# ChrisTho23/DrakeGPT

Measured on NVIDIA B200. Metric: train_tokens_per_sec_TransformerLM_scaled, higher is better.
Workload: dtype bf16

## Files before the change

drakegpt_b200/csrc/attn_tc.cu:

```cuda
#include <cuda.h>

#include "common.cuh"
#include "ptx.cuh"

namespace dgpt {

using namespace ptx;

int make_tmap_bf16_2d(CUtensorMap* map, const void* base, int64_t inner, int64_t outer, int64_t ld, int box_outer);

static constexpr int HD = 64;
static constexpr int QT = 128;
static constexpr float kLog2e = 1.4426950408889634f;

struct AttnTcP {
  void *o, *dq, *dk, *dv;
  const void *o_in, *d_o;
  float* lse;
  int64_t o_rs, dq_rs, dk_rs, dv_rs, do_rs;
  int B, NH, T;
  float scale, inv_keep;
  uint32_t thr, site;
  uint64_t seed;
  const uint64_t* seed_dev;
};

__device__ __forceinline__ uint32_t pack_bf16(float a, float b) {
  __nv_bfloat162 v = __floats2bfloat162_rn(a, b);
  return *reinterpret_cast<uint32_t*>(&v);
}

__device__ __forceinline__ void store_row32_sw128(uint8_t* tile_base, int row, int c0, const float (&v)[32]) {
  uint8_t* blk = tile_base + (c0 >> 6) * 16384 + row * 128;
  const int chunk0 = (c0 & 63) >> 3;
#pragma unroll
  for (int j = 0; j < 4; ++j) {
    uint4 w;
    w.x = pack_bf16(v[8 * j], v[8 * j + 1]);
    w.y = pack_bf16(v[8 * j + 2], v[8 * j + 3]);
    w.z = pack_bf16(v[8 * j + 4], v[8 * j + 5]);
    w.w = pack_bf16(v[8 * j + 6], v[8 * j + 7]);
    *reinterpret_cast<uint4*>(blk + (((chunk0 + j) ^ (row & 7)) << 4)) = w;
  }
}

static constexpr int kFwd2Threads = 320;
static constexpr int kFwd2QK = 49152;
static constexpr int kFwd2Smem = 2 * kFwd2QK + 2 * 32768 + 256 + 1024;
static constexpr int kWHeavy = 5, kWLight = 2;

struct FwdSched {
  int nheavy, nlight;
  unsigned long long* probe;
};

__global__ void __launch_bounds__(kFwd2Threads, 1)
attn_fwd_tc2_kernel(const __grid_constant__ CUtensorMap map_q32, const __grid_constant__ CUtensorMap map_k,
                    const __grid_constant__ CUtensorMap map_v, AttnTcP p, FwdSched sc) {
  extern __shared__ uint8_t smem_raw[];
  uint8_t* smem = reinterpret_cast<uint8_t*>((reinterpret_cast<uintptr_t>(smem_raw) + 1023) & ~(uintptr_t)1023);
  uint8_t* sQK = smem;
  uint8_t* sV = smem + 2 * kFwd2QK;
  uint64_t* bars = reinterpret_cast<uint64_t*>(sV + 2 * 32768);
  uint64_t *qk_full = bars, *qk_empty = bars + 2, *v_full = bars + 4, *v_empty = bars + 6, *s_full = bars + 8,
           *p_full = bars + 10, *o_full = bars + 12, *slot_free = bars + 14;
  uint32_t* tmem_slot = reinterpret_cast<uint32_t*>(bars + 16);

  clock_probe_begin(sc.probe);
  const int warp = threadIdx.x >> 5, lane = threadIdx.x & 31;
  const int ntile = p.T / QT;

  const int G = gridDim.x, c = blockIdx.x;
  const int hq = sc.nheavy / G, hr = sc.nheavy % G;
  const int nh_c = hq + (c < hr ? 1 : 0);
  const int U = (kWHeavy * sc.nheavy + kWLight * sc.nlight + G - 1) / G;
  const int cap_hi = max(0, (U - kWHeavy * (hq + 1)) / kWLight), cap_lo = max(0, (U - kWHeavy * hq) / kWLight);
  const int cap_total = hr * cap_hi + (G - hr) * cap_lo;
  const int l_start = c < hr ? c * cap_hi : hr * cap_hi + (c - hr) * cap_lo;
  const int l0 = min(sc.nlight, l_start), l1 = min(sc.nlight, l_start + (c < hr ? cap_hi : cap_lo));
  const int n_extra = cap_total < sc.nlight ? (sc.nlight - cap_total - c + G - 1) / G : 0;
  const int n_items = nh_c + (l1 - l0) + max(0, n_extra);
  auto item = [&](int n, int& bh, int& qt) {
    if (n < nh_c) {
      const int hi = c + n * G;
      bh = hi; qt = ntile - 1;
    } else {
      const int m = n - nh_c;
      const int li = m < l1 - l0 ? l0 + m : cap_total + c + (m - (l1 - l0)) * G;
      bh = li; qt = 0;
    }
  };

  if (threadIdx.x == 0) {
    prefetch_tensormap(&map_q32);
    prefetch_tensormap(&map_k);
    prefetch_tensormap(&map_v);
    for (int g = 0; g < 2; ++g) {
      mbar_init(&qk_full[g], 1);
      mbar_init(&qk_empty[g], 1);
      mbar_init(&v_full[g], 1);
      mbar_init(&v_empty[g], 1);
      mbar_init(&s_full[g], 1);
      mbar_init(&p_full[g], 4);
      mbar_init(&o_full[g], 1);
      mbar_init(&slot_free[g], 4);
    }
    fence_barrier_init();
  }
  if (warp == 9) tmem_alloc<512>(tmem_slot);
  tc_fence_before();
  __syncthreads();
  tc_fence_after();
  const uint32_t tmem = *tmem_slot;
  pdl_grid_sync();

  if (warp == 8) {
    for (int n = 0; n < n_items; ++n) {
      const int g = n & 1, k = n >> 1;
      int bh, qt;
      item(n, bh, qt);
      const int nkv = qt + 1, b = bh / p.NH, h = bh % p.NH, row0 = b * p.T;
      uint8_t* q_s = sQK + g * kFwd2QK;
      uint8_t* v_s = sV + g * 32768;
      mbar_wait(&qk_empty[g], (k & 1) ^ 1);
      if (elect_one()) {
        mbar_expect_tx(&qk_full[g], 16384 * (1 + nkv));
        for (int qb = 0; qb < 4; ++qb)
          tma_load_2d(q_s + qb * 4096, &map_q32, &qk_full[g], h * HD, row0 + qt * QT + (g ? 3 - qb : qb) * 32);
        for (int j = 0; j < nkv; ++j) tma_load_2d(q_s + 16384 * (1 + j), &map_k, &qk_full[g], h * HD, row0 + j * QT);
      }
      __syncwarp();
      mbar_wait(&v_empty[g], (k & 1) ^ 1);
      if (elect_one()) {
        mbar_expect_tx(&v_full[g], 16384 * nkv);
        for (int kb = 0; kb < 2 * nkv; ++kb) tma_load_2d(v_s + kb * 8192, &map_v, &v_full[g], h * HD, row0 + kb * 64);
      }
      __syncwarp();
    }
  } else if (warp == 9) {
    constexpr uint32_t idesc_s = make_idesc_bf16(128, 128, 0, 0);
    constexpr uint32_t idesc_o = make_idesc_bf16(128, 64, 0, 1);
    int next_s = 0, next_pv = 0;
    while (next_pv < n_items) {
      bool progressed = false;
      if (next_s < n_items) {
        const int g = next_s & 1, k = next_s >> 1;
        if (mbar_test(&qk_full[g], k & 1) && mbar_test(&slot_free[g], (k & 1) ^ 1)) {
          tc_fence_after();
          int bh, qt;
          item(next_s, bh, qt);
          const int nkv = qt + 1;
          const uint64_t dq0 = make_smem_desc_sw128(smem_u32(sQK + g * kFwd2QK), 16, 1024);
          const uint64_t dk0 = make_smem_desc_sw128(smem_u32(sQK + g * kFwd2QK + 16384), 16, 1024);
          if (elect_one()) {
            for (int j = 0; j < nkv; ++j) {
#pragma unroll
              for (int kk = 0; kk < 4; ++kk)
                tc_mma_bf16(tmem + g * 256 + j * 128, dq0 + (uint64_t)(kk * 2), dk0 + (uint64_t)(j * 1024 + kk * 2), idesc_s, kk > 0);
            }
            tc_commit(&s_full[g]);
            tc_commit(&qk_empty[g]);
          }
          __syncwarp();
          ++next_s;
          progressed = true;
        }
      }
      if (next_pv < next_s) {
        const int g = next_pv & 1, k = next_pv >> 1;
        if (mbar_test(&p_full[g], k & 1) && mbar_test(&v_full[g], k & 1)) {
          tc_fence_after();
          int bh, qt;
          item(next_pv, bh, qt);
          const int nkv = qt + 1;
          const uint64_t dv0 = make_smem_desc_sw128(smem_u32(sV + g * 32768), 8192, 1024);
          if (elect_one()) {
            for (int kb = 0; kb < 2 * nkv; ++kb) {
#pragma unroll
              for (int kk = 0; kk < 4; ++kk)
                tc_mma_bf16_ts(tmem + g * 256 + nkv * 64, tmem + g * 256 + kb * 32 + kk * 8, dv0 + (uint64_t)(kb * 512 + kk * 128),
                               idesc_o, (kb | kk) > 0);
            }
            tc_commit(&o_full[g]);
            tc_commit(&v_empty[g]);
          }
          __syncwarp();
          ++next_pv;
          progressed = true;
        }
      }
      if (!progressed) __nanosleep(32);
    }
  } else {
    const int g = warp >> 2;
    const int quad = warp & 3;
    const int rblk = g ? 3 - quad : quad;
    const int row = rblk * 32 + lane;
    const uint32_t taddr = tmem + (uint32_t)(g * 256) + ((uint32_t)(quad * 32) << 16);
    uint64_t seed = p.seed;
    if (p.thr && p.seed_dev) seed += *p.seed_dev;
    const float sc2 = p.scale * kLog2e;
    for (int n = g; n < n_items; n += 2) {
      const int k = n >> 1;
      int bh, qt;
      item(n, bh, qt);
      const int nkv = qt + 1, b = bh / p.NH, h = bh % p.NH, row0 = b * p.T;
      const int qg = qt * QT + row;
      const int ncols = nkv * QT;
#define FTS(i) do { if (sc.probe && blockIdx.x == 0 && warp == 0 && lane == 0 && k < 3) sc.probe[4 + k * 8 + (i)] = (unsigned long long)clock64(); } while (0)
      FTS(0);
      mbar_wait(&s_full[g], k & 1);
      FTS(1);
      tc_fence_after();
      const int qg_max = qt * QT + rblk * 32 + 31, qg_min = qt * QT + rblk * 32;
      float mx = -INFINITY;
      for (int cc = 0; cc < ncols && cc <= qg_max; cc += 32) {
        uint32_t r[32];
        tmem_ld32(taddr + cc, r);
        tmem_ld_wait();
        if (cc + 31 <= qg_min) {
#pragma unroll
          for (int j = 0; j < 32; ++j) mx = fmaxf(mx, __uint_as_float(r[j]));
        } else {
#pragma unroll
          for (int j = 0; j < 32; ++j)
            if (cc + j <= qg) mx = fmaxf(mx, __uint_as_float(r[j]));
        }
      }
      FTS(2);
      const float msc = mx * sc2;
      float sum = 0.f;
      const uint64_t base = (((uint64_t)b * p.NH + h) * p.T + qg) * (uint64_t)p.T;
      for (int cc = 0; cc < ncols; cc += 32) {
        float e[32];
        if (cc > qg_max) {
#pragma unroll
          for (int j = 0; j < 32; ++j) e[j] = 0.f;
        } else {
          uint32_t r[32];
          tmem_ld32(taddr + cc, r);
          tmem_ld_wait();
          if (cc + 31 <= qg_min) {
#pragma unroll
            for (int j = 0; j < 32; ++j) {
              const float v = exp2f(__uint_as_float(r[j]) * sc2 - msc);
              sum += v;
              e[j] = v;
            }
          } else {
#pragma unroll
            for (int j = 0; j < 32; ++j) {
              const float v = (cc + j <= qg) ? exp2f(__uint_as_float(r[j]) * sc2 - msc) : 0.f;
              sum += v;
              e[j] = v;
            }
          }
          if (p.thr) {
            const DropGroup dg = dropout_group(seed, p.site, (base + cc) >> 5);
#pragma unroll
            for (int j = 0; j < 32; ++j)
              if (dropout_word(dg, j) < p.thr) e[j] = 0.f;
          }
        }
        uint32_t pk[16];
#pragma unroll
        for (int j = 0; j < 16; ++j) pk[j] = pack_bf16(e[2 * j], e[2 * j + 1]);
        tmem_st16(taddr + (cc >> 1), pk);
      }
      if (p.lse) p.lse[((int64_t)b * p.NH + h) * p.T + qg] = mx * p.scale + logf(sum);
      tmem_st_wait();
      tc_fence_before();
      __syncwarp();
      if (lane == 0) mbar_arrive(&p_full[g]);
      FTS(3);
      mbar_wait(&o_full[g], k & 1);
      FTS(4);
      tc_fence_after();
      const float oscale = p.inv_keep / sum;
      __nv_bfloat16* orow = reinterpret_cast<__nv_bfloat16*>(p.o) + (int64_t)(row0 + qg) * p.o_rs + h * HD;
#pragma unroll
      for (int cc = 0; cc < HD; cc += 32) {
        uint32_t r[32];
        tmem_ld32(taddr + nkv * 64 + cc, r);
        tmem_ld_wait();
#pragma unroll
        for (int j = 0; j < 4; ++j) {
          uint4 w;
          w.x = pack_bf16(__uint_as_float(r[8 * j]) * oscale, __uint_as_float(r[8 * j + 1]) * oscale);
          w.y = pack_bf16(__uint_as_float(r[8 * j + 2]) * oscale, __uint_as_float(r[8 * j + 3]) * oscale);
          w.z = pack_bf16(__uint_as_float(r[8 * j + 4]) * oscale, __uint_as_float(r[8 * j + 5]) * oscale);
          w.w = pack_bf16(__uint_as_float(r[8 * j + 6]) * oscale, __uint_as_float(r[8 * j + 7]) * oscale);
          *reinterpret_cast<uint4*>(orow + cc + 8 * j) = w;
        }
      }
      tc_fence_before();
      __syncwarp();
      if (lane == 0) mbar_arrive(&slot_free[g]);
      FTS(5);
    }
  }
  tc_fence_before();
  __syncthreads();
  if (warp == 9) {
    tc_fence_after();
    tmem_dealloc<512>(tmem);
  }
  clock_probe_end(sc.probe);
}

#ifdef DGPT_ATTN_TS
__device__ long long g_attn_ts[64];
#endif
static constexpr int kBwdThreads = 64 + 256;
static constexpr int kBwdSmem = 8 * 16384 + 2 * 32768 + 16384 + 2048 + 1024 + 128;

template <bool DIAG, bool DROP>
__device__ __forceinline__ void bwd_chunk_math(const AttnTcP& p, uint32_t lane_addr_st, uint32_t lane_addr_dp, int row, int k0,
                                               float sc, float lse2, float Dq, uint64_t seed, uint64_t base,
                                               float (&pd)[32], float (&ds)[32]) {
  uint32_t st[32], dp[32];
  tmem_ld32(lane_addr_st + k0, st);
  tmem_ld32(lane_addr_dp + k0, dp);
  tmem_ld_wait();
  DropGroup g = {0u, 0u};
  if (DROP) g = dropout_group(seed, p.site, (base + k0) >> 5);
#pragma unroll
  for (int t = 0; t < 32; ++t) {
    float pv = exp2f(__uint_as_float(st[t]) * sc - lse2);
    if (DIAG) pv = (k0 + t) <= row ? pv : 0.f;
    float dpv = __uint_as_float(dp[t]);
    float pdv = pv;
    if (DROP) {
      const bool keep = dropout_word(g, t) >= p.thr;
      dpv = keep ? dpv * p.inv_keep : 0.f;
      pdv = keep ? pv * p.inv_keep : 0.f;
    }
    pd[t] = pdv;
    ds[t] = pv * (dpv - Dq) * p.scale;
  }
}

template <bool DROP>
__global__ void __launch_bounds__(kBwdThreads, 1)
attn_bwd_tc_kernel(const __grid_constant__ CUtensorMap map_q, const __grid_constant__ CUtensorMap map_k,
                   const __grid_constant__ CUtensorMap map_v, const __grid_constant__ CUtensorMap map_do,
                   const __grid_constant__ CUtensorMap map_o, const __grid_constant__ CUtensorMap map_dq,
                   const __grid_constant__ CUtensorMap map_dk, const __grid_constant__ CUtensorMap map_dv, AttnTcP p) {
  extern __shared__ __align__(1024) uint8_t smem[];
  uint8_t* sQ = smem;
  uint8_t* sK = smem + 2 * 16384;
  uint8_t* sV = smem + 4 * 16384;
  uint8_t* sG = smem + 6 * 16384;
  uint8_t* sPd = smem + 8 * 16384;
  uint8_t* sDs = sPd + 32768;
  uint8_t* sSt = sDs + 32768;
  float* lse_s = reinterpret_cast<float*>(sSt + 16384);
  float* D_s = lse_s + 256;
  uint64_t* bars = reinterpret_cast<uint64_t*>(D_s + 256);
  uint64_t *ld_a = bars, *st_full = bars + 1, *ps_full = bars + 2, *drained = bars + 3, *acc_done = bars + 4;
  uint64_t *ld_b = bars + 5, *ld_c = bars + 6;
  uint64_t* acc_free = bars + 7;
  uint32_t* tmem_slot = reinterpret_cast<uint32_t*>(bars + 8);

  const int warp = threadIdx.x >> 5, lane = threadIdx.x & 31;
#ifdef DGPT_ATTN_TS
#define BTS(i) do { if (blockIdx.x == 0 && blockIdx.y == (gridDim.y / 2) && warp == 2 && lane == 0) g_attn_ts[i] = clock64(); } while (0)
#else
#define BTS(i) do { } while (0)
#endif
  BTS(0);
  const int h = blockIdx.x, b = blockIdx.y;
  const int ntile = p.T / QT;
  const int npair = ntile == 1 ? 1 : 3;
  const int row0 = b * p.T;

  if (threadIdx.x == 0) {
    prefetch_tensormap(&map_q);
    prefetch_tensormap(&map_k);
    prefetch_tensormap(&map_v);
    prefetch_tensormap(&map_do);
    prefetch_tensormap(&map_o);
    mbar_init(ld_a, 1);
    mbar_init(ld_b, 1);
    mbar_init(ld_c, 1);
    mbar_init(st_full, 1);
    mbar_init(ps_full, 8);
    mbar_init(drained, 8);
    mbar_init(acc_done, 1);
    mbar_init(acc_free, 1);
    fence_barrier_init();
  }
  if (warp == 0) {
    __syncwarp();
    pdl_grid_sync();
    if (elect_one()) {
      mbar_expect_tx(ld_a, 16384 * 5);
      tma_load_2d(sG, &map_do, ld_a, h * HD, row0);
      tma_load_2d(sPd, &map_o, ld_a, h * HD, row0);
      tma_load_2d(sQ, &map_q, ld_a, h * HD, row0);
      tma_load_2d(sK, &map_k, ld_a, h * HD, row0);
      tma_load_2d(sV, &map_v, ld_a, h * HD, row0);
      if (ntile > 1) {
        mbar_expect_tx(ld_b, 16384 * 3);
        tma_load_2d(sG + 16384, &map_do, ld_b, h * HD, row0 + QT);
        tma_load_2d(sSt, &map_o, ld_b, h * HD, row0 + QT);
        tma_load_2d(sQ + 16384, &map_q, ld_b, h * HD, row0 + QT);
        mbar_expect_tx(ld_c, 16384 * 2);
        tma_load_2d(sK + 16384, &map_k, ld_c, h * HD, row0 + QT);
        tma_load_2d(sV + 16384, &map_v, ld_c, h * HD, row0 + QT);
      }
    }
  }
  if (warp == 1) tmem_alloc<512>(tmem_slot);
  tc_fence_before();
  __syncthreads();
  tc_fence_after();
  const uint32_t tmem = *tmem_slot;
  constexpr uint32_t TM_ST = 0, TM_DP = 128, TM_DV = 256, TM_DK = 320, TM_DQ = 384;
  if (warp != 0) pdl_grid_sync();

  if (warp == 0) {
  } else if (warp == 1) {
    constexpr uint32_t id_kk = make_idesc_bf16(128, 128, 0, 0);
    constexpr uint32_t id_kmn = make_idesc_bf16(128, 64, 0, 1);
    constexpr uint32_t id_mnmn = make_idesc_bf16(128, 64, 1, 1);
    mbar_wait(ld_a, 0);
    tc_fence_after();
    const uint64_t kQ = make_smem_desc_sw128(smem_u32(sQ), 16, 1024), kK = make_smem_desc_sw128(smem_u32(sK), 16, 1024);
    const uint64_t kV = make_smem_desc_sw128(smem_u32(sV), 16, 1024), kG = make_smem_desc_sw128(smem_u32(sG), 16, 1024);
    const uint64_t kDs = make_smem_desc_sw128(smem_u32(sDs), 16, 1024);
    const uint64_t mQ = make_smem_desc_sw128(smem_u32(sQ), 8192, 1024), mK = make_smem_desc_sw128(smem_u32(sK), 8192, 1024);
    const uint64_t mG = make_smem_desc_sw128(smem_u32(sG), 8192, 1024);
    const uint64_t mPd = make_smem_desc_sw128(smem_u32(sPd), 16384, 1024), mDs = make_smem_desc_sw128(smem_u32(sDs), 16384, 1024);
    auto issue_s_dp = [&](int pr) {
      const int i = pr == 0 ? 0 : 1, j = pr == 2 ? 1 : 0;
      if (elect_one()) {
#pragma unroll
        for (int k = 0; k < 4; ++k)
          tc_mma_bf16(tmem + TM_ST, kQ + (uint64_t)(i * 1024 + k * 2), kK + (uint64_t)(j * 1024 + k * 2), id_kk, k > 0);
#pragma unroll
        for (int k = 0; k < 4; ++k)
          tc_mma_bf16(tmem + TM_DP, kG + (uint64_t)(i * 1024 + k * 2), kV + (uint64_t)(j * 1024 + k * 2), id_kk, k > 0);
        tc_commit(st_full);
      }
      __syncwarp();
    };
    issue_s_dp(0);
    for (int pr = 0; pr < npair; ++pr) {
      const int i = pr == 0 ? 0 : 1, j = pr == 2 ? 1 : 0;
      mbar_wait(ps_full, pr & 1);
      if (pr + 1 < npair) {
        mbar_wait(pr + 1 == 1 ? ld_b : ld_c, 0);
        tc_fence_after();
        issue_s_dp(pr + 1);
      }
      if (pr > 0) mbar_wait(drained, (pr - 1) & 1);
      tc_fence_after();
      const uint32_t acc_vk = (pr == 1) ? 1u : 0u;
      const uint32_t acc_q = (pr == 2) ? 1u : 0u;
      if (elect_one()) {
#pragma unroll
        for (int k = 0; k < 8; ++k)
          tc_mma_bf16(tmem + TM_DV, mPd + (uint64_t)(k * 128), mG + (uint64_t)(i * 1024 + k * 128), id_mnmn, acc_vk | (k > 0));
#pragma unroll
        for (int k = 0; k < 8; ++k)
          tc_mma_bf16(tmem + TM_DK, mDs + (uint64_t)(k * 128), mQ + (uint64_t)(i * 1024 + k * 128), id_mnmn, acc_vk | (k > 0));
#pragma unroll
        for (int k = 0; k < 8; ++k)
          tc_mma_bf16(tmem + TM_DQ, kDs + (uint64_t)((k >> 2) * 1024 + (k & 3) * 2), mK + (uint64_t)(j * 1024 + k * 128), id_kmn,
                      acc_q | (k > 0));
        tc_commit(acc_free);
        if (pr == npair - 1) tc_commit(acc_done);
      }
      __syncwarp();
    }
  } else {
    const int cw = warp - 2;
    const int quad = warp & 3;
    const int half = cw >> 2;
    const int rowl = quad * 32 + lane;
    const int ct = threadIdx.x - 64;
    const uint32_t lane_addr = tmem + ((uint32_t)(quad * 32) << 16);
    uint64_t seed = p.seed;
    if (DROP && p.seed_dev) seed += *p.seed_dev;
    if (ct < p.T) lse_s[ct] = p.lse[((int64_t)b * p.NH + h) * p.T + ct] * kLog2e;
    auto compute_D = [&](int tl, const uint8_t* o_tile) {
      if (ct < QT) {
        const int r = ct;
        const uint8_t* gr = sG + tl * 16384 + r * 128;
        const uint8_t* orow = o_tile + r * 128;
        float acc = 0.f;
#pragma unroll
        for (int c = 0; c < 8; ++c) {
          const int off = (c ^ (r & 7)) << 4;
          const uint4 g = *reinterpret_cast<const uint4*>(gr + off), o = *reinterpret_cast<const uint4*>(orow + off);
          const uint32_t gw[4] = {g.x, g.y, g.z, g.w}, ow[4] = {o.x, o.y, o.z, o.w};
#pragma unroll
          for (int t = 0; t < 4; ++t) {
            const float2 gf = __bfloat1622float2(*reinterpret_cast<const __nv_bfloat162*>(&gw[t]));
            const float2 of = __bfloat1622float2(*reinterpret_cast<const __nv_bfloat162*>(&ow[t]));
            acc = fmaf(gf.x, of.x, acc);
            acc = fmaf(gf.y, of.y, acc);
          }
        }
        D_s[tl * QT + r] = acc;
      }
      asm volatile("bar.sync 1, 256;" ::: "memory");
    };
    BTS(1);
    mbar_wait(ld_a, 0);
    BTS(2);
    compute_D(0, sPd);
    const float sc = p.scale * kLog2e;
    int n_stores = 0;

    auto drain = [&](uint32_t tm_col, const CUtensorMap* map, int tile) {
      uint32_t r[32];
      tmem_ld32(lane_addr + tm_col + half * 32, r);
      if (n_stores > 0) {
        if (ct == 0) bulk_wait_read<0>();
        asm volatile("bar.sync 1, 256;" ::: "memory");
      }
      tmem_ld_wait();
      uint8_t* rp = sSt + rowl * 128;
#pragma unroll
      for (int j = 0; j < 4; ++j) {
        uint4 w;
        w.x = pack_bf16(__uint_as_float(r[8 * j]), __uint_as_float(r[8 * j + 1]));
        w.y = pack_bf16(__uint_as_float(r[8 * j + 2]), __uint_as_float(r[8 * j + 3]));
        w.z = pack_bf16(__uint_as_float(r[8 * j + 4]), __uint_as_float(r[8 * j + 5]));
        w.w = pack_bf16(__uint_as_float(r[8 * j + 6]), __uint_as_float(r[8 * j + 7]));
        *reinterpret_cast<uint4*>(rp + (((half * 4 + j) ^ (rowl & 7)) << 4)) = w;
      }
      fence_proxy_async();
      asm volatile("bar.sync 1, 256;" ::: "memory");
      if (ct == 0) {
        tma_store_2d(map, sSt, h * HD, row0 + tile * QT);
        bulk_commit();
      }
      ++n_stores;
    };

    BTS(3);
    for (int pr = 0; pr < npair; ++pr) {
      const int i = pr == 0 ? 0 : 1, j = pr == 2 ? 1 : 0;
      if (pr == 1) {
        mbar_wait(ld_b, 0);
        compute_D(1, sSt);
      }
      BTS(4 + 4 * pr);
      mbar_wait(st_full, pr & 1);
      BTS(5 + 4 * pr);
      tc_fence_after();
      const int qi = i * QT + rowl;
      const float lse2 = lse_s[qi], Dq = D_s[qi];
      const uint64_t base = (((uint64_t)b * p.NH + h) * p.T + qi) * (uint64_t)p.T + (uint64_t)(j * QT);
      float pd[32], ds[32];
      if (i == j) bwd_chunk_math<true, DROP>(p, lane_addr + TM_ST, lane_addr + TM_DP, rowl, half * 64, sc, lse2, Dq, seed, base, pd, ds);
      else bwd_chunk_math<false, DROP>(p, lane_addr + TM_ST, lane_addr + TM_DP, rowl, half * 64, sc, lse2, Dq, seed, base, pd, ds);
      if (pr > 0) {
        mbar_wait(acc_free, (pr - 1) & 1);
        tc_fence_after();
        if (pr == 1) {
          drain(TM_DQ, &map_dq, 0);
        } else {
          drain(TM_DV, &map_dv, 0);
          drain(TM_DK, &map_dk, 0);
        }
        tc_fence_before();
        __syncwarp();
        if (lane == 0) mbar_arrive(drained);
      }
      BTS(6 + 4 * pr);
      store_row32_sw128(sPd, rowl, half * 64, pd);
      store_row32_sw128(sDs, rowl, half * 64, ds);
      if (i == j) bwd_chunk_math<true, DROP>(p, lane_addr + TM_ST, lane_addr + TM_DP, rowl, half * 64 + 32, sc, lse2, Dq, seed, base, pd, ds);
      else bwd_chunk_math<false, DROP>(p, lane_addr + TM_ST, lane_addr + TM_DP, rowl, half * 64 + 32, sc, lse2, Dq, seed, base, pd, ds);
      store_row32_sw128(sPd, rowl, half * 64 + 32, pd);
      store_row32_sw128(sDs, rowl, half * 64 + 32, ds);
      fence_proxy_async();
      tc_fence_before();
      __syncwarp();
      if (lane == 0) mbar_arrive(ps_full);
      BTS(7 + 4 * pr);
    }
    BTS(16);
    mbar_wait(acc_done, 0);
    BTS(17);
    tc_fence_after();
    const int last = ntile - 1;
    {
      if (n_stores > 0) {
        if (ct == 0) bulk_wait_read<0>();
        asm volatile("bar.sync 1, 256;" ::: "memory");
      }
      uint8_t* tiles[3] = {sPd, sDs, sSt};
      const uint32_t cols[3] = {TM_DV, TM_DK, TM_DQ};
#pragma unroll
      for (int q = 0; q < 3; ++q) {
        uint32_t r[32];
        tmem_ld32(lane_addr + cols[q] + half * 32, r);
        tmem_ld_wait();
        uint8_t* rp = tiles[q] + rowl * 128;
#pragma unroll
        for (int j = 0; j < 4; ++j) {
          uint4 w;
          w.x = pack_bf16(__uint_as_float(r[8 * j]), __uint_as_float(r[8 * j + 1]));
          w.y = pack_bf16(__uint_as_float(r[8 * j + 2]), __uint_as_float(r[8 * j + 3]));
          w.z = pack_bf16(__uint_as_float(r[8 * j + 4]), __uint_as_float(r[8 * j + 5]));
          w.w = pack_bf16(__uint_as_float(r[8 * j + 6]), __uint_as_float(r[8 * j + 7]));
          *reinterpret_cast<uint4*>(rp + (((half * 4 + j) ^ (rowl & 7)) << 4)) = w;
        }
      }
      fence_proxy_async();
      asm volatile("bar.sync 1, 256;" ::: "memory");
      if (ct == 0) {
        tma_store_2d(&map_dv, sPd, h * HD, row0 + last * QT);
        tma_store_2d(&map_dk, sDs, h * HD, row0 + last * QT);
        tma_store_2d(&map_dq, sSt, h * HD, row0 + last * QT);
        bulk_commit();
      }
    }
    if (ct == 0) bulk_wait<0>();
    BTS(18);
  }
  tc_fence_before();
  __syncthreads();
  if (warp == 1) {
    tc_fence_after();
    tmem_dealloc<512>(tmem);
  }
}

bool attn_tc_supported(const dgpt_attn_args* a) {
  if (a->dtype != DGPT_BF16 || a->H != HD || a->Tq != a->Tk) return false;
  if (a->Tk != 128 && a->Tk != 256) return false;
  const int64_t T = a->Tk;
  auto ok = [&](const void* ptr, int64_t bs, int64_t rs) {
    return ptr && ((uintptr_t)ptr & 15) == 0 && rs % 8 == 0 && bs == T * rs;
  };
  if (!ok(a->q, a->q_bs, a->q_rs) || !ok(a->k, a->k_bs, a->k_rs) || !ok(a->v, a->v_bs, a->v_rs) ||
      !ok(a->o, a->o_bs, a->o_rs))
    return false;
  if (a->d_o) {
    if (!ok(a->d_o, a->do_bs, a->do_rs) || !ok(a->dq, a->dq_bs, a->dq_rs) || !ok(a->dk, a->dk_bs, a->dk_rs) ||
        !ok(a->dv, a->dv_bs, a->dv_rs) || !a->lse)
      return false;
  }
  return true;
}

static AttnTcP make_tc_params(const dgpt_attn_args* a) {
  AttnTcP p;
  p.o = a->o; p.dq = a->dq; p.dk = a->dk; p.dv = a->dv; p.o_in = a->o; p.d_o = a->d_o; p.lse = a->lse;
  p.o_rs = a->o_rs; p.dq_rs = a->dq_rs; p.dk_rs = a->dk_rs; p.dv_rs = a->dv_rs; p.do_rs = a->do_rs;
  p.B = a->B; p.NH = a->NH; p.T = a->Tk;
  p.scale = a->scale; p.inv_keep = 1.f / (1.f - a->dropout_p);
  p.thr = dropout_threshold(a->dropout_p); p.site = a->site; p.seed = a->seed; p.seed_dev = a->seed_dev;
  return p;
}

int launch_attn_fwd_tc(const dgpt_attn_args* a, cudaStream_t st) {
  CUtensorMap mq, mk, mv;
  const int64_t rows = (int64_t)a->B * a->Tk, cols = (int64_t)a->NH * HD;
  int rc;
  if ((rc = make_tmap_bf16_2d(&mq, a->q, cols, rows, a->q_rs, 32))) return rc;
  if ((rc = make_tmap_bf16_2d(&mk, a->k, cols, rows, a->k_rs, QT))) return rc;
  if ((rc = make_tmap_bf16_2d(&mv, a->v, cols, rows, a->v_rs, 64))) return rc;
  AttnTcP p = make_tc_params(a);
  static bool attr = false;
  if (!attr) {
    cudaError_t e = cudaFuncSetAttribute(attn_fwd_tc2_kernel, cudaFuncAttributeMaxDynamicSharedMemorySize, kFwd2Smem);
    if (e != cudaSuccess) { set_error("attn_fwd_tc2: smem attribute: %s", cudaGetErrorString(e)); return DGPT_E_LAUNCH; }
    attr = true;
  }
  const int ntile = a->Tk / QT, bh = a->B * a->NH;
  FwdSched sc;
  sc.nheavy = ntile > 1 ? bh : 0;
  sc.nlight = bh;
  sc.probe = clock_probe_buffer();
  int sms = dgpt_sm_count();
  if (sms <= 0) sms = 148;
  const int grid = min(sms, sc.nheavy + sc.nlight);
  launch_pdl(attn_fwd_tc2_kernel, dim3(grid), dim3(kFwd2Threads), kFwd2Smem, st, mq, mk, mv, p, sc);
  return check_launch("attn_fwd_tc2");
}

int launch_attn_bwd_tc(const dgpt_attn_args* a, cudaStream_t st) {
  CUtensorMap mq, mk, mv, mg, mo, mdq, mdk, mdv;
  const int64_t rows = (int64_t)a->B * a->Tk, cols = (int64_t)a->NH * HD;
  int rc;
  if ((rc = make_tmap_bf16_2d(&mq, a->q, cols, rows, a->q_rs, QT))) return rc;
  if ((rc = make_tmap_bf16_2d(&mk, a->k, cols, rows, a->k_rs, QT))) return rc;
  if ((rc = make_tmap_bf16_2d(&mv, a->v, cols, rows, a->v_rs, QT))) return rc;
  if ((rc = make_tmap_bf16_2d(&mg, a->d_o, cols, rows, a->do_rs, QT))) return rc;
  if ((rc = make_tmap_bf16_2d(&mo, a->o, cols, rows, a->o_rs, QT))) return rc;
  if ((rc = make_tmap_bf16_2d(&mdq, a->dq, cols, rows, a->dq_rs, QT))) return rc;
  if ((rc = make_tmap_bf16_2d(&mdk, a->dk, cols, rows, a->dk_rs, QT))) return rc;
  if ((rc = make_tmap_bf16_2d(&mdv, a->dv, cols, rows, a->dv_rs, QT))) return rc;
  static bool attr = false;
  if (!attr) {
    cudaError_t e = cudaFuncSetAttribute(attn_bwd_tc_kernel<true>, cudaFuncAttributeMaxDynamicSharedMemorySize, kBwdSmem);
    if (e == cudaSuccess)
      e = cudaFuncSetAttribute(attn_bwd_tc_kernel<false>, cudaFuncAttributeMaxDynamicSharedMemorySize, kBwdSmem);
    if (e != cudaSuccess) { set_error("attn_bwd_tc: smem attribute: %s", cudaGetErrorString(e)); return DGPT_E_LAUNCH; }
    attr = true;
  }
  AttnTcP p = make_tc_params(a);
  dim3 grid(a->NH, a->B);
  if (p.thr) launch_pdl(attn_bwd_tc_kernel<true>, grid, dim3(kBwdThreads), kBwdSmem, st, mq, mk, mv, mg, mo, mdq, mdk, mdv, p);
  else launch_pdl(attn_bwd_tc_kernel<false>, grid, dim3(kBwdThreads), kBwdSmem, st, mq, mk, mv, mg, mo, mdq, mdk, mdv, p);
#ifdef DGPT_ATTN_TS
  {
    cudaStreamSynchronize(st);
    long long h[64];
    cudaMemcpyFromSymbol(h, g_attn_ts, sizeof(h));
    printf("attn bwd CTA: setup %lld | load wait %lld | D %lld |", h[1] - h[0], h[2] - h[1], h[3] - h[2]);
    for (int pr = 0; pr < 3; ++pr)
      printf(" pair%d: S/dP wait %lld, drains %lld, chunks %lld |", pr, h[5 + 4 * pr] - h[4 + 4 * pr], h[6 + 4 * pr] - h[5 + 4 * pr],
             h[7 + 4 * pr] - h[6 + 4 * pr]);
    printf(" acc wait %lld | final drains %lld | total %lld\n", h[17] - h[16], h[18] - h[17], h[18] - h[0]);
    fflush(stdout);
  }
#endif
  return check_launch("attn_bwd_tc");
}

}
```

Before: 7.834 million.

## Make attention backward kernel persistent with cross-item load prefetch and register-computed D

Turns the attention backward kernel from a one-CTA-per-(batch,head) grid into a persistent grid capped at the SM count. Each CTA loops over several items and prefetches the next item's Q/K/V/dO tiles via TMA while the current item's MMAs and drains finish, with a new a_free barrier and parity tracking across items. The D = rowsum(dO·O) term and LSE are now computed from global loads with warp shuffles into double-buffered shared arrays, which drops the O tensor-map TMA load into shared memory. This targets wave quantization, launch/setup overhead and load latency, at the cost of more complex barrier phase logic and uncoalesced __ldg reads.

```diff
diff --git a/drakegpt_b200/csrc/attn_tc.cu b/drakegpt_b200/csrc/attn_tc.cu
--- a/drakegpt_b200/csrc/attn_tc.cu
+++ b/drakegpt_b200/csrc/attn_tc.cu
@@ -24,6 +24,12 @@
   uint64_t seed;
   const uint64_t* seed_dev;
 };
+
+__device__ __forceinline__ int warp_id() {
+  uint32_t t;
+  asm volatile("mov.u32 %0, %%tid.x;" : "=r"(t));
+  return (int)(t >> 5);
+}
 
 __device__ __forceinline__ uint32_t pack_bf16(float a, float b) {
   __nv_bfloat162 v = __floats2bfloat162_rn(a, b);
@@ -310,9 +316,11 @@
 
 #ifdef DGPT_ATTN_TS
 __device__ long long g_attn_ts[64];
+__device__ unsigned long long g_attn_cta[2 * 1024];
 #endif
 static constexpr int kBwdThreads = 64 + 256;
-static constexpr int kBwdSmem = 8 * 16384 + 2 * 32768 + 16384 + 2048 + 1024 + 128;
+static constexpr int kBwdTsItem = 20;
+static constexpr int kBwdSmem = 8 * 16384 + 2 * 32768 + 16384 + 2 * 2048 + 1024 + 128;
 
 template <bool DIAG, bool DROP>
 __device__ __forceinline__ void bwd_chunk_math(const AttnTcP& p, uint32_t lane_addr_st, uint32_t lane_addr_dp, int row, int k0,
@@ -324,10 +332,11 @@
   tmem_ld_wait();
   DropGroup g = {0u, 0u};
   if (DROP) g = dropout_group(seed, p.site, (base + k0) >> 5);
+  const int tmax = row - k0;
 #pragma unroll
   for (int t = 0; t < 32; ++t) {
     float pv = exp2f(__uint_as_float(st[t]) * sc - lse2);
-    if (DIAG) pv = (k0 + t) <= row ? pv : 0.f;
+    if (DIAG) pv = t <= tmax ? pv : 0.f;
     float dpv = __uint_as_float(dp[t]);
     float pdv = pv;
     if (DROP) {
@@ -344,8 +353,8 @@
 __global__ void __launch_bounds__(kBwdThreads, 1)
 attn_bwd_tc_kernel(const __grid_constant__ CUtensorMap map_q, const __grid_constant__ CUtensorMap map_k,
                    const __grid_constant__ CUtensorMap map_v, const __grid_constant__ CUtensorMap map_do,
-                   const __grid_constant__ CUtensorMap map_o, const __grid_constant__ CUtensorMap map_dq,
-                   const __grid_constant__ CUtensorMap map_dk, const __grid_constant__ CUtensorMap map_dv, AttnTcP p) {
+                   const __grid_constant__ CUtensorMap map_dq, const __grid_constant__ CUtensorMap map_dk,
+                   const __grid_constant__ CUtensorMap map_dv, AttnTcP p) {
   extern __shared__ __align__(1024) uint8_t smem[];
   uint8_t* sQ = smem;
   uint8_t* sK = smem + 2 * 16384;
@@ -355,61 +364,76 @@
   uint8_t* sDs = sPd + 32768;
   uint8_t* sSt = sDs + 32768;
   float* lse_s = reinterpret_cast<float*>(sSt + 16384);
-  float* D_s = lse_s + 256;
-  uint64_t* bars = reinterpret_cast<uint64_t*>(D_s + 256);
-  uint64_t *ld_a = bars, *st_full = bars + 1, *ps_full = bars + 2, *drained = bars + 3, *acc_done = bars + 4;
-  uint64_t *ld_b = bars + 5, *ld_c = bars + 6;
-  uint64_t* acc_free = bars + 7;
-  uint32_t* tmem_slot = reinterpret_cast<uint32_t*>(bars + 8);
+  float* D_s = lse_s + 512;
+  uint64_t* bars = reinterpret_cast<uint64_t*>(D_s + 512);
+  uint64_t *ld_a = bars, *ld_b = bars + 1, *ld_c = bars + 2, *st_full = bars + 3, *ps_full = bars + 4;
+  uint64_t *acc_free = bars + 5, *a_free = bars + 6, *acc_done = bars + 7, *drained = bars + 8;
+  uint32_t* tmem_slot = reinterpret_cast<uint32_t*>(bars + 9);
 
   const int warp = threadIdx.x >> 5, lane = threadIdx.x & 31;
 #ifdef DGPT_ATTN_TS
-#define BTS(i) do { if (blockIdx.x == 0 && blockIdx.y == (gridDim.y / 2) && warp == 2 && lane == 0) g_attn_ts[i] = clock64(); } while (0)
+#define BTS(n, i) do { if (blockIdx.x == 0 && warp == 2 && lane == 0 && (n) < 3) g_attn_ts[(n) * kBwdTsItem + (i)] = clock64(); } while (0)
 #else
-#define BTS(i) do { } while (0)
+#define BTS(n, i) do { } while (0)
 #endif
-  BTS(0);
-  const int h = blockIdx.x, b = blockIdx.y;
+  BTS(0, 0);
+#ifdef DGPT_ATTN_TS
+  if (threadIdx.x == 0) g_attn_cta[2 * blockIdx.x] = global_timer_ns();
+#endif
   const int ntile = p.T / QT;
   const int npair = ntile == 1 ? 1 : 3;
-  const int row0 = b * p.T;
+  const int n_items = (p.B * p.NH - (int)blockIdx.x + (int)gridDim.x - 1) / (int)gridDim.x;
+  auto item_bh = [&](int n, int& b, int& h) {
+    const int it = (int)blockIdx.x + n * (int)gridDim.x;
+    b = it / p.NH;
+    h = it % p.NH;
+  };
 
   if (threadIdx.x == 0) {
     prefetch_tensormap(&map_q);
     prefetch_tensormap(&map_k);
     prefetch_tensormap(&map_v);
     prefetch_tensormap(&map_do);
-    prefetch_tensormap(&map_o);
     mbar_init(ld_a, 1);
     mbar_init(ld_b, 1);
     mbar_init(ld_c, 1);
     mbar_init(st_full, 1);
     mbar_init(ps_full, 8);
+    mbar_init(acc_free, 1);
+    mbar_init(a_free, 1);
+    mbar_init(acc_done, 1);
     mbar_init(drained, 8);
-    mbar_init(acc_done, 1);
-    mbar_init(acc_free, 1);
     fence_barrier_init();
   }
+  auto load_a = [&](int n) {
+    int b, h;
+    item_bh(n, b, h);
+    const int row0 = b * p.T;
+    mbar_expect_tx(ld_a, 16384 * 4);
+    tma_load_2d(sG, &map_do, ld_a, h * HD, row0);
+    tma_load_2d(sQ, &map_q, ld_a, h * HD, row0);
+    tma_load_2d(sK, &map_k, ld_a, h * HD, row0);
+    tma_load_2d(sV, &map_v, ld_a, h * HD, row0);
+  };
+  auto load_bc = [&](int n) {
+    int b, h;
+    item_bh(n, b, h);
+    const int row0 = b * p.T;
+    mbar_expect_tx(ld_b, 16384 * 2);
+    tma_load_2d(sG + 16384, &map_do, ld_b, h * HD, row0 + QT);
+    tma_load_2d(sQ + 16384, &map_q, ld_b, h * HD, row0 + QT);
+    mbar_expect_tx(ld_c, 16384 * 2);
+    tma_load_2d(sK + 16384, &map_k, ld_c, h * HD, row0 + QT);
+    tma_load_2d(sV + 16384, &map_v, ld_c, h * HD, row0 + QT);
+  };
   if (warp == 0) {
     __syncwarp();
     pdl_grid_sync();
     if (elect_one()) {
-      mbar_expect_tx(ld_a, 16384 * 5);
-      tma_load_2d(sG, &map_do, ld_a, h * HD, row0);
-      tma_load_2d(sPd, &map_o, ld_a, h * HD, row0);
-      tma_load_2d(sQ, &map_q, ld_a, h * HD, row0);
-      tma_load_2d(sK, &map_k, ld_a, h * HD, row0);
-      tma_load_2d(sV, &map_v, ld_a, h * HD, row0);
-      if (ntile > 1) {
-        mbar_expect_tx(ld_b, 16384 * 3);
-        tma_load_2d(sG + 16384, &map_do, ld_b, h * HD, row0 + QT);
-        tma_load_2d(sSt, &map_o, ld_b, h * HD, row0 + QT);
-        tma_load_2d(sQ + 16384, &map_q, ld_b, h * HD, row0 + QT);
-        mbar_expect_tx(ld_c, 16384 * 2);
-        tma_load_2d(sK + 16384, &map_k, ld_c, h * HD, row0 + QT);
-        tma_load_2d(sV + 16384, &map_v, ld_c, h * HD, row0 + QT);
-      }
-    }
+      load_a(0);
+      if (ntile > 1) load_bc(0);
+    }
+    __syncwarp();
   }
   if (warp == 1) tmem_alloc<512>(tmem_slot);
   tc_fence_before();
@@ -420,12 +444,20 @@
   if (warp != 0) pdl_grid_sync();
 
   if (warp == 0) {
+    for (int n = 1; n < n_items; ++n) {
+      mbar_wait(a_free, (n - 1) & 1);
+      if (elect_one()) load_a(n);
+      __syncwarp();
+      if (ntile > 1) {
+        mbar_wait(acc_done, (n - 1) & 1);
+        if (elect_one()) load_bc(n);
+        __syncwarp();
+      }
+    }
   } else if (warp == 1) {
     constexpr uint32_t id_kk = make_idesc_bf16(128, 128, 0, 0);
     constexpr uint32_t id_kmn = make_idesc_bf16(128, 64, 0, 1);
     constexpr uint32_t id_mnmn = make_idesc_bf16(128, 64, 1, 1);
-    mbar_wait(ld_a, 0);
-    tc_fence_after();
     const uint64_t kQ = make_smem_desc_sw128(smem_u32(sQ), 16, 1024), kK = make_smem_desc_sw128(smem_u32(sK), 16, 1024);
     const uint64_t kV = make_smem_desc_sw128(smem_u32(sV), 16, 1024), kG = make_smem_desc_sw128(smem_u32(sG), 16, 1024);
     const uint64_t kDs = make_smem_desc_sw128(smem_u32(sDs), 16, 1024);
@@ -445,34 +477,45 @@
       }
       __syncwarp();
     };
+    mbar_wait(ld_a, 0);
+    tc_fence_after();
     issue_s_dp(0);
-    for (int pr = 0; pr < npair; ++pr) {
-      const int i = pr == 0 ? 0 : 1, j = pr == 2 ? 1 : 0;
-      mbar_wait(ps_full, pr & 1);
-      if (pr + 1 < npair) {
-        mbar_wait(pr + 1 == 1 ? ld_b : ld_c, 0);
+    for (int n = 0; n < n_items; ++n) {
+      for (int pr = 0; pr < npair; ++pr) {
+        const int i = pr == 0 ? 0 : 1, j = pr == 2 ? 1 : 0;
+        const int k = n * npair + pr;
+        mbar_wait(ps_full, k & 1);
+        if (pr + 1 < npair) {
+          mbar_wait(pr + 1 == 1 ? ld_b : ld_c, n & 1);
+          tc_fence_after();
+          issue_s_dp(pr + 1);
+        }
+        if (k > 0) mbar_wait(drained, (k - 1) & 1);
         tc_fence_after();
-        issue_s_dp(pr + 1);
-      }
-      if (pr > 0) mbar_wait(drained, (pr - 1) & 1);
-      tc_fence_after();
-      const uint32_t acc_vk = (pr == 1) ? 1u : 0u;
-      const uint32_t acc_q = (pr == 2) ? 1u : 0u;
-      if (elect_one()) {
-#pragma unroll
-        for (int k = 0; k < 8; ++k)
-          tc_mma_bf16(tmem + TM_DV, mPd + (uint64_t)(k * 128), mG + (uint64_t)(i * 1024 + k * 128), id_mnmn, acc_vk | (k > 0));
-#pragma unroll
-        for (int k = 0; k < 8; ++k)
-          tc_mma_bf16(tmem + TM_DK, mDs + (uint64_t)(k * 128), mQ + (uint64_t)(i * 1024 + k * 128), id_mnmn, acc_vk | (k > 0));
-#pragma unroll
-        for (int k = 0; k < 8; ++k)
-          tc_mma_bf16(tmem + TM_DQ, kDs + (uint64_t)((k >> 2) * 1024 + (k & 3) * 2), mK + (uint64_t)(j * 1024 + k * 128), id_kmn,
-                      acc_q | (k > 0));
-        tc_commit(acc_free);
-        if (pr == npair - 1) tc_commit(acc_done);
-      }
-      __syncwarp();
+        const uint32_t acc_vk = (pr == 1) ? 1u : 0u;
+        const uint32_t acc_q = (pr == 2) ? 1u : 0u;
+        if (elect_one()) {
+#pragma unroll
+          for (int kk = 0; kk < 8; ++kk)
+            tc_mma_bf16(tmem + TM_DV, mPd + (uint64_t)(kk * 128), mG + (uint64_t)(i * 1024 + kk * 128), id_mnmn, acc_vk | (kk > 0));
+#pragma unroll
+          for (int kk = 0; kk < 8; ++kk)
+            tc_mma_bf16(tmem + TM_DK, mDs + (uint64_t)(kk * 128), mQ + (uint64_t)(i * 1024 + kk * 128), id_mnmn, acc_vk | (kk > 0));
+#pragma unroll
+          for (int kk = 0; kk < 8; ++kk)
+            tc_mma_bf16(tmem + TM_DQ, kDs + (uint64_t)((kk >> 2) * 1024 + (kk & 3) * 2), mK + (uint64_t)(j * 1024 + kk * 128),
+                        id_kmn, acc_q | (kk > 0));
+          tc_commit(acc_free);
+          if (pr == (npair == 1 ? 0 : 1)) tc_commit(a_free);
+          if (pr == npair - 1) tc_commit(acc_done);
+        }
+        __syncwarp();
+      }
+      if (n + 1 < n_items) {
+        mbar_wait(ld_a, (n + 1) & 1);
+        tc_fence_after();
+        issue_s_dp(0);
+      }
     }
   } else {
     const int cw = warp - 2;
@@ -483,36 +526,55 @@
     const uint32_t lane_addr = tmem + ((uint32_t)(quad * 32) << 16);
     uint64_t seed = p.seed;
     if (DROP && p.seed_dev) seed += *p.seed_dev;
-    if (ct < p.T) lse_s[ct] = p.lse[((int64_t)b * p.NH + h) * p.T + ct] * kLog2e;
-    auto compute_D = [&](int tl, const uint8_t* o_tile) {
-      if (ct < QT) {
-        const int r = ct;
-        const uint8_t* gr = sG + tl * 16384 + r * 128;
-        const uint8_t* orow = o_tile + r * 128;
-        float acc = 0.f;
-#pragma unroll
-        for (int c = 0; c < 8; ++c) {
-          const int off = (c ^ (r & 7)) << 4;
-          const uint4 g = *reinterpret_cast<const uint4*>(gr + off), o = *reinterpret_cast<const uint4*>(orow + off);
-          const uint32_t gw[4] = {g.x, g.y, g.z, g.w}, ow[4] = {o.x, o.y, o.z, o.w};
-#pragma unroll
-          for (int t = 0; t < 4; ++t) {
-            const float2 gf = __bfloat1622float2(*reinterpret_cast<const __nv_bfloat162*>(&gw[t]));
-            const float2 of = __bfloat1622float2(*reinterpret_cast<const __nv_bfloat162*>(&ow[t]));
-            acc = fmaf(gf.x, of.x, acc);
-            acc = fmaf(gf.y, of.y, acc);
+    auto load_stats = [&](int n) {
+      int b, h;
+      item_bh(n, b, h);
+      if (cw * 32 < p.T) {
+        const int q = lane & 3, rw = cw * 32 + (lane >> 2);
+        const int64_t r0 = (int64_t)b * p.T + rw;
+        const __nv_bfloat16* gb = reinterpret_cast<const __nv_bfloat16*>(p.d_o) + r0 * p.do_rs + h * HD + q * 16;
+        const __nv_bfloat16* ob = reinterpret_cast<const __nv_bfloat16*>(p.o_in) + r0 * p.o_rs + h * HD + q * 16;
+        uint4 g[4][2], o[4][2];
+#pragma unroll
+        for (int i = 0; i < 4; ++i) {
+#pragma unroll
+          for (int k = 0; k < 2; ++k) {
+            g[i][k] = __ldg(reinterpret_cast<const uint4*>(gb + (int64_t)i * 8 * p.do_rs) + k);
+            o[i][k] = __ldg(reinterpret_cast<const uint4*>(ob + (int64_t)i * 8 * p.o_rs) + k);
           }
         }
-        D_s[tl * QT + r] = acc;
-      }
-      asm volatile("bar.sync 1, 256;" ::: "memory");
+        const float l = p.lse[((int64_t)b * p.NH + h) * p.T + cw * 32 + lane];
+        float acc[4] = {0.f, 0.f, 0.f, 0.f};
+#pragma unroll
+        for (int s = 0; s < 4; ++s) {
+#pragma unroll
+          for (int i = 0; i < 4; ++i) {
+            float a = s == 0 ? 0.f : __shfl_up_sync(0xffffffffu, acc[i], 1);
+#pragma unroll
+            for (int k = 0; k < 2; ++k) {
+              const uint32_t gw[4] = {g[i][k].x, g[i][k].y, g[i][k].z, g[i][k].w};
+              const uint32_t ow[4] = {o[i][k].x, o[i][k].y, o[i][k].z, o[i][k].w};
+#pragma unroll
+              for (int t = 0; t < 4; ++t) {
+                const float2 gf = __bfloat1622float2(*reinterpret_cast<const __nv_bfloat162*>(&gw[t]));
+                const float2 of = __bfloat1622float2(*reinterpret_cast<const __nv_bfloat162*>(&ow[t]));
+                a = fmaf(gf.x, of.x, a);
+                a = fmaf(gf.y, of.y, a);
+              }
+            }
+            if (q == s) acc[i] = a;
+          }
+        }
+        if (q == 3) {
+#pragma unroll
+          for (int i = 0; i < 4; ++i) D_s[(n & 1) * 256 + rw + 8 * i] = acc[i];
+        }
+        lse_s[(n & 1) * 256 + cw * 32 + lane] = l * kLog2e;
+      }
     };
-    BTS(1);
-    mbar_wait(ld_a, 0);
-    BTS(2);
-    compute_D(0, sPd);
     const float sc = p.scale * kLog2e;
     int n_stores = 0;
+    int h = 0, row0 = 0;
 
     auto drain = [&](uint32_t tm_col, const CUtensorMap* map, int tile) {
       uint32_t r[32];
@@ -541,92 +603,111 @@
       ++n_stores;
     };
 
-    BTS(3);
-    for (int pr = 0; pr < npair; ++pr) {
-      const int i = pr == 0 ? 0 : 1, j = pr == 2 ? 1 : 0;
-      if (pr == 1) {
-        mbar_wait(ld_b, 0);
-        compute_D(1, sSt);
-      }
-      BTS(4 + 4 * pr);
-      mbar_wait(st_full, pr & 1);
-      BTS(5 + 4 * pr);
+    load_stats(0);
+    asm volatile("bar.sync 1, 256;" ::: "memory");
+    for (int n = 0; n < n_items; ++n) {
+      if (n > 0) BTS(n, 0);
+      BTS(n, 3);
+      int b;
+      item_bh(n, b, h);
+      row0 = b * p.T;
+      const float* lse_n = lse_s + (n & 1) * 256;
+      const float* D_n = D_s + (n & 1) * 256;
+      for (int pr = 0; pr < npair; ++pr) {
+        const int i = pr == 0 ? 0 : 1, j = pr == 2 ? 1 : 0;
+        const int k = n * npair + pr;
+        BTS(n, 4 + 4 * pr);
+        mbar_wait(st_full, k & 1);
+        BTS(n, 5 + 4 * pr);
+        tc_fence_after();
+        const int qi = i * QT + rowl;
+        const float lse2 = lse_n[qi], Dq = D_n[qi];
+        const uint64_t base = (((uint64_t)b * p.NH + h) * p.T + qi) * (uint64_t)p.T + (uint64_t)(j * QT);
+        float pd[32], ds[32];
+        if (i == j) bwd_chunk_math<true, DROP>(p, lane_addr + TM_ST, lane_addr + TM_DP, rowl, half * 64, sc, lse2, Dq, seed, base, pd, ds);
+        else bwd_chunk_math<false, DROP>(p, lane_addr + TM_ST, lane_addr + TM_DP, rowl, half * 64, sc, lse2, Dq, seed, base, pd, ds);
+        if (pr > 0) {
+          mbar_wait(acc_free, (k - 1) & 1);
+          tc_fence_after();
+          if (pr == 1) {
+            drain(TM_DQ, &map_dq, 0);
+          } else {
+            drain(TM_DV, &map_dv, 0);
+            drain(TM_DK, &map_dk, 0);
+          }
+          tc_fence_before();
+          __syncwarp();
+          if (lane == 0) mbar_arrive(drained);
+        } else if (n > 0) {
+          if (ct == 0) bulk_wait_read<0>();
+          asm volatile("bar.sync 1, 256;" ::: "memory");
+        }
+        BTS(n, 6 + 4 * pr);
+        store_row32_sw128(sPd, rowl, half * 64, pd);
+        store_row32_sw128(sDs, rowl, half * 64, ds);
+        if (i == j) bwd_chunk_math<true, DROP>(p, lane_addr + TM_ST, lane_addr + TM_DP, rowl, half * 64 + 32, sc, lse2, Dq, seed, base, pd, ds);
+        else bwd_chunk_math<false, DROP>(p, lane_addr + TM_ST, lane_addr + TM_DP, rowl, half * 64 + 32, sc, lse2, Dq, seed, base, pd, ds);
+        store_row32_sw128(sPd, rowl, half * 64 + 32, pd);
+        store_row32_sw128(sDs, rowl, half * 64 + 32, ds);
+        fence_proxy_async();
+        tc_fence_before();
+        __syncwarp();
+        if (lane == 0) mbar_arrive(ps_full);
+        BTS(n, 7 + 4 * pr);
+      }
+      BTS(n, 16);
+      if (n + 1 < n_items) load_stats(n + 1);
+      BTS(n, 17);
+      mbar_wait(acc_done, n & 1);
+      BTS(n, 18);
       tc_fence_after();
-      const int qi = i * QT + rowl;
-      const float lse2 = lse_s[qi], Dq = D_s[qi];
-      const uint64_t base = (((uint64_t)b * p.NH + h) * p.T + qi) * (uint64_t)p.T + (uint64_t)(j * QT);
-      float pd[32], ds[32];
-      if (i == j) bwd_chunk_math<true, DROP>(p, lane_addr + TM_ST, lane_addr + TM_DP, rowl, half * 64, sc, lse2, Dq, seed, base, pd, ds);
-      else bwd_chunk_math<false, DROP>(p, lane_addr + TM_ST, lane_addr + TM_DP, rowl, half * 64, sc, lse2, Dq, seed, base, pd, ds);
-      if (pr > 0) {
-        mbar_wait(acc_free, (pr - 1) & 1);
-        tc_fence_after();
-        if (pr == 1) {
-          drain(TM_DQ, &map_dq, 0);
-        } else {
-          drain(TM_DV, &map_dv, 0);
-          drain(TM_DK, &map_dk, 0);
+      const int last = ntile - 1;
+      {
+        if (n_stores > 0) {
+          if (ct == 0) bulk_wait_read<0>();
+          asm volatile("bar.sync 1, 256;" ::: "memory");
+        }
+        uint8_t* tiles[3] = {sPd, sDs, sSt};
+        const uint32_t cols[3] = {TM_DV, TM_DK, TM_DQ};
+#pragma unroll
+        for (int q = 0; q < 3; ++q) {
+          uint32_t r[32];
+          tmem_ld32(lane_addr + cols[q] + half * 32, r);
+          tmem_ld_wait();
+          uint8_t* rp = tiles[q] + rowl * 128;
+#pragma unroll
+          for (int j = 0; j < 4; ++j) {
+            uint4 w;
+            w.x = pack_bf16(__uint_as_float(r[8 * j]), __uint_as_float(r[8 * j + 1]));
+            w.y = pack_bf16(__uint_as_float(r[8 * j + 2]), __uint_as_float(r[8 * j + 3]));
+            w.z = pack_bf16(__uint_as_float(r[8 * j + 4]), __uint_as_float(r[8 * j + 5]));
+            w.w = pack_bf16(__uint_as_float(r[8 * j + 6]), __uint_as_float(r[8 * j + 7]));
+            *reinterpret_cast<uint4*>(rp + (((half * 4 + j) ^ (rowl & 7)) << 4)) = w;
+          }
         }
         tc_fence_before();
         __syncwarp();
         if (lane == 0) mbar_arrive(drained);
-      }
-      BTS(6 + 4 * pr);
-      store_row32_sw128(sPd, rowl, half * 64, pd);
-      store_row32_sw128(sDs, rowl, half * 64, ds);
-      if (i == j) bwd_chunk_math<true, DROP>(p, lane_addr + TM_ST, lane_addr + TM_DP, rowl, half * 64 + 32, sc, lse2, Dq, seed, base, pd, ds);
-      else bwd_chunk_math<false, DROP>(p, lane_addr + TM_ST, lane_addr + TM_DP, rowl, half * 64 + 32, sc, lse2, Dq, seed, base, pd, ds);
-      store_row32_sw128(sPd, rowl, half * 64 + 32, pd);
-      store_row32_sw128(sDs, rowl, half * 64 + 32, ds);
-      fence_proxy_async();
-      tc_fence_before();
-      __syncwarp();
-      if (lane == 0) mbar_arrive(ps_full);
-      BTS(7 + 4 * pr);
-    }
-    BTS(16);
-    mbar_wait(acc_done, 0);
-    BTS(17);
-    tc_fence_after();
-    const int last = ntile - 1;
-    {
-      if (n_stores > 0) {
-        if (ct == 0) bulk_wait_read<0>();
+        fence_proxy_async();
         asm volatile("bar.sync 1, 256;" ::: "memory");
-      }
-      uint8_t* tiles[3] = {sPd, sDs, sSt};
-      const uint32_t cols[3] = {TM_DV, TM_DK, TM_DQ};
-#pragma unroll
-      for (int q = 0; q < 3; ++q) {
-        uint32_t r[32];
-        tmem_ld32(lane_addr + cols[q] + half * 32, r);
-        tmem_ld_wait();
-        uint8_t* rp = tiles[q] + rowl * 128;
-#pragma unroll
-        for (int j = 0; j < 4; ++j) {
-          uint4 w;
-          w.x = pack_bf16(__uint_as_float(r[8 * j]), __uint_as_float(r[8 * j + 1]));
-          w.y = pack_bf16(__uint_as_float(r[8 * j + 2]), __uint_as_float(r[8 * j + 3]));
-          w.z = pack_bf16(__uint_as_float(r[8 * j + 4]), __uint_as_float(r[8 * j + 5]));
-          w.w = pack_bf16(__uint_as_float(r[8 * j + 6]), __uint_as_float(r[8 * j + 7]));
-          *reinterpret_cast<uint4*>(rp + (((half * 4 + j) ^ (rowl & 7)) << 4)) = w;
-        }
-      }
-      fence_proxy_async();
-      asm volatile("bar.sync 1, 256;" ::: "memory");
-      if (ct == 0) {
-        tma_store_2d(&map_dv, sPd, h * HD, row0 + last * QT);
-        tma_store_2d(&map_dk, sDs, h * HD, row0 + last * QT);
-        tma_store_2d(&map_dq, sSt, h * HD, row0 + last * QT);
-        bulk_commit();
-      }
+        if (ct == 0) {
+          tma_store_2d(&map_dv, sPd, h * HD, row0 + last * QT);
+          tma_store_2d(&map_dk, sDs, h * HD, row0 + last * QT);
+          tma_store_2d(&map_dq, sSt, h * HD, row0 + last * QT);
+          bulk_commit();
+        }
+        n_stores += 3;
+      }
+      BTS(n, 19);
     }
     if (ct == 0) bulk_wait<0>();
-    BTS(18);
   }
   tc_fence_before();
   __syncthreads();
-  if (warp == 1) {
+#ifdef DGPT_ATTN_TS
+  if (threadIdx.x == 0) g_attn_cta[2 * blockIdx.x + 1] = global_timer_ns();
+#endif
+  if (warp_id() == 1) {
     tc_fence_after();
     tmem_dealloc<512>(tmem);
   }
@@ -687,14 +768,13 @@
 }
 
 int launch_attn_bwd_tc(const dgpt_attn_args* a, cudaStream_t st) {
-  CUtensorMap mq, mk, mv, mg, mo, mdq, mdk, mdv;
+  CUtensorMap mq, mk, mv, mg, mdq, mdk, mdv;
   const int64_t rows = (int64_t)a->B * a->Tk, cols = (int64_t)a->NH * HD;
   int rc;
   if ((rc = make_tmap_bf16_2d(&mq, a->q, cols, rows, a->q_rs, QT))) return rc;
   if ((rc = make_tmap_bf16_2d(&mk, a->k, cols, rows, a->k_rs, QT))) return rc;
   if ((rc = make_tmap_bf16_2d(&mv, a->v, cols, rows, a->v_rs, QT))) return rc;
   if ((rc = make_tmap_bf16_2d(&mg, a->d_o, cols, rows, a->do_rs, QT))) return rc;
-  if ((rc = make_tmap_bf16_2d(&mo, a->o, cols, rows, a->o_rs, QT))) return rc;
   if ((rc = make_tmap_bf16_2d(&mdq, a->dq, cols, rows, a->dq_rs, QT))) return rc;
   if ((rc = make_tmap_bf16_2d(&mdk, a->dk, cols, rows, a->dk_rs, QT))) return rc;
   if ((rc = make_tmap_bf16_2d(&mdv, a->dv, cols, rows, a->dv_rs, QT))) return rc;
@@ -707,19 +787,39 @@
     attr = true;
   }
   AttnTcP p = make_tc_params(a);
-  dim3 grid(a->NH, a->B);
-  if (p.thr) launch_pdl(attn_bwd_tc_kernel<true>, grid, dim3(kBwdThreads), kBwdSmem, st, mq, mk, mv, mg, mo, mdq, mdk, mdv, p);
-  else launch_pdl(attn_bwd_tc_kernel<false>, grid, dim3(kBwdThreads), kBwdSmem, st, mq, mk, mv, mg, mo, mdq, mdk, mdv, p);
+  int sms = dgpt_sm_count();
+  if (sms <= 0) sms = 148;
+  const int n_all = a->B * a->NH;
+  const dim3 grid(min(sms, n_all));
+  if (p.thr) launch_pdl(attn_bwd_tc_kernel<true>, grid, dim3(kBwdThreads), kBwdSmem, st, mq, mk, mv, mg, mdq, mdk, mdv, p);
+  else launch_pdl(attn_bwd_tc_kernel<false>, grid, dim3(kBwdThreads), kBwdSmem, st, mq, mk, mv, mg, mdq, mdk, mdv, p);
 #ifdef DGPT_ATTN_TS
   {
     cudaStreamSynchronize(st);
     long long h[64];
     cudaMemcpyFromSymbol(h, g_attn_ts, sizeof(h));
-    printf("attn bwd CTA: setup %lld | load wait %lld | D %lld |", h[1] - h[0], h[2] - h[1], h[3] - h[2]);
-    for (int pr = 0; pr < 3; ++pr)
-      printf(" pair%d: S/dP wait %lld, drains %lld, chunks %lld |", pr, h[5 + 4 * pr] - h[4 + 4 * pr], h[6 + 4 * pr] - h[5 + 4 * pr],
-             h[7 + 4 * pr] - h[6 + 4 * pr]);
-    printf(" acc wait %lld | final drains %lld | total %lld\n", h[17] - h[16], h[18] - h[17], h[18] - h[0]);
+    const int npair = a->Tk == 256 ? 3 : 1, n0 = min(3, (n_all + (int)grid.x - 1) / (int)grid.x);
+    for (int n = 0; n < n0; ++n) {
+      const long long* t = h + n * kBwdTsItem;
+      printf("attn bwd CTA 0 item %d: start +%lld | %s %lld |", n, t[0] - h[0], n == 0 ? "setup + lse/D" : "-", t[3] - t[0]);
+      for (int pr = 0; pr < npair; ++pr)
+        printf(" pair%d: S/dP wait %lld, drains %lld, chunks %lld |", pr, t[5 + 4 * pr] - t[4 + 4 * pr], t[6 + 4 * pr] - t[5 + 4 * pr],
+               t[7 + 4 * pr] - t[6 + 4 * pr]);
+      printf(" next lse/D %lld | acc wait %lld | final drains %lld | total %lld\n", t[17] - t[16], t[18] - t[17], t[19] - t[18],
+             t[19] - t[0]);
+    }
+    static unsigned long long c[2 * 1024];
+    cudaMemcpyFromSymbol(c, g_attn_cta, sizeof(unsigned long long) * 2 * grid.x);
+    unsigned long long t0 = ~0ull, s_max = 0, e_max[4] = {0, 0, 0, 0}, e_min = ~0ull;
+    for (unsigned g = 0; g < grid.x; ++g) t0 = min(t0, c[2 * g]);
+    for (unsigned g = 0; g < grid.x; ++g) {
+      const int ni = min(3, (n_all - (int)g + (int)grid.x - 1) / (int)grid.x);
+      s_max = max(s_max, c[2 * g] - t0);
+      e_max[ni] = max(e_max[ni], c[2 * g + 1] - t0);
+      e_min = min(e_min, c[2 * g + 1] - t0);
+    }
+    printf("attn bwd CTAs (ns from the first start): last start %llu | first end %llu | last end, CTAs of 1 / 2 / 3 items: %llu %llu %llu\n",
+           s_max, e_min, e_max[1], e_max[2], e_max[3]);
     fflush(stdout);
   }
 #endif
```

Result: no change. 7.852 million, median of 6 (+0.2%).
